# LiHaoxu/SpMV-Research

Measured on AMD Instinct MI355X. Metric: GFLOP/s (2*nnz/t, fp64 SpMV y=A*x); achieved HBM GB/s and % of peak in 'roofline', higher is better.
Workload: dtype f64; 1 GPU; nlpkkt240 (synthetic twin); format=MI355X_SELLD_64_16384_d_v7, rows=27993600, cols=27993600, nnz=765374392, parallelism=single GPU

## Files before the change

### spmv-research_amd/csrc/build_sell.hip

```cpp
#include "handle.hpp"

namespace spmv {

static std::vector<int>
sigma_sort(const int * rp, long m, long sigma)
{
	std::vector<int> row_of_sorted(std::max<long>(m, 1));
	const long num_windows = (m + sigma - 1) / sigma;
	#pragma omp parallel for num_threads(spmv::host_threads()) schedule(dynamic, 4)
	for (long w = 0; w < num_windows; w++)
	{
		long s = w * sigma, e = std::min(m, s + sigma);
		int maxlen = 0;
		for (long i = s; i < e; i++)
			maxlen = std::max(maxlen, rp[i + 1] - rp[i]);
		std::vector<long> cnt((size_t) maxlen + 2, 0);
		for (long i = s; i < e; i++)
			cnt[maxlen - (rp[i + 1] - rp[i]) + 1]++;
		for (int b = 0; b <= maxlen; b++)
			cnt[b + 1] += cnt[b];
		for (long i = s; i < e; i++)
			row_of_sorted[s + cnt[maxlen - (rp[i + 1] - rp[i])]++] = (int) i;
	}
	return row_of_sorted;
// ... 517 lines not shown
			long js = 0, len = 0;
			if (i < m)
			{
				const int o = row_of_sorted[i];
				js = rp[o];
				len = rp[o + 1] - rp[o];
			}
			const unsigned short pad = (len > 0 && !sym) ? (unsigned short) (ci[js + len - 1] - lo) : (unsigned short) gw;
			for (long k = 0; k < width; k++)
			{
				val[(size_t) (vb + sellw_val_pos(k, r, A->f32))] = k < len ? va[js + k] : 0.0;
				idx[(size_t) (ib + (k / 4) * 4 * C + r * 4 + k % 4)] = k < len ? (unsigned short) (ci[js + k] - lo) : pad;
			}
		}
	}
	A->sell_slices = num_slices;
	A->sell_nnz_ext = nnz_ext;
	A->sell_idx_bytes = idx_count * 2;
	A->sellw_groups = (int) num_groups;
	A->sellw_ns = NS;
	A->sell_split = S;
	A->sellw_lds = (int) (((long) (max_w + 1) * A->vbytes + 15) / 16 * 16);
	A->sellw_wmax = max_w;
	{
		std::vector<int64_t> gp((size_t) num_groups + 1, 0);
		for (long g = 0; g < num_groups; g++)
			gp[(size_t) g + 1] = sdesc[2 * std::min<long>(num_slices, (g + 1) * NS)];
		A->cfg.map = xcd_map_balanced(gp.data(), num_groups, 1, resolve_remap(A->remap, num_groups));
	}
	if (upload_ints(grp.data(), grp.size(), &A->d_sellw_grp) || dev_alloc(&A->d_sell_desc, sdesc.size()))
		return 1;
	HIP_TRY(hipMemcpy(A->d_sell_desc, sdesc.data(), sdesc.size() * sizeof(int64_t), hipMemcpyHostToDevice));
	if (upload_bytes(idx.data(), (size_t) idx_count * 2, 1024, (void **) &A->d_sell_idx) || upload_values(A, val.data(), (size_t) nnz_ext, &A->d_val) ||
	    upload_ints(row_of_sorted.data(), (size_t) m, &A->d_row_of_sorted))
		return 1;
	A->mem_footprint = (double) (num_slices + 1) * 16 + (double) num_groups * 16 + (double) nnz_ext * A->vbytes + (double) idx_count * 2 + (double) m * 4;
	return 0;
}

int
build_sell_symmetric(spmv_mi355x_matrix * A, const spmv_mi355x_opts & o, const int * rp, const int * ci, const double * va)
{
	const long lm = A->m;
	const long slices = (lm + 63) / 64;
	const char * pf = A->f32 ? "f" : "d";
	int S = o.sell_split ? o.sell_split : (slices >= 8192 ? 1 : slices >= 2048 ? 2 : 4);
	int NS = o.sell_group ? o.sell_group : 16 / S;
	if ((S != 1 && S != 2 && S != 4) || NS < 1 || NS * S > 16 || (NS & (NS - 1)))
		return 2;
	A->sell_c = 64;
	A->sell_delta = false;
	A->convert_on_device = o.convert_on != 2 && !getenv("SPMV_MI355X_HOST_CONVERT");
	const int took = build_sell_window(A, rp, ci, va, NS, S, 152 * 1024, true);
	if (took)
		return took;
	A->sell_window = true;
	A->sell_sym = true;
	A->sell_sigma = 64L * NS;
	if (o.nontemporal == 0)
		A->cfg.nt = (double) A->sell_nnz_ext * (A->vbytes + 2) > 32.0 * 1024 * 1024 ? 1 : 0;
	if (S > 1)
		snprintf(A->format_name, sizeof(A->format_name), "MI355X_SELLWS_64_%d_w%d_%s", 64 * NS, S, pf);
	else
		snprintf(A->format_name, sizeof(A->format_name), "MI355X_SELLWS_64_%d_%s", 64 * NS, pf);
	snprintf(A->kernel_name, sizeof(A->kernel_name), "sell_window_sym_kernel");
	A->kernel_block = 64 * NS * S;
	return 0;
}

int
build_sell_family(spmv_mi355x_matrix * A, const spmv_mi355x_opts & o, const int * rp, const int * ci, const double * va)
{
	const long lm = A->m;
	const char * pf = A->f32 ? "f" : "d";
	int rc = 0;
	int C = o.sell_c ? o.sell_c : 64;
	if (C != 16 && C != 32 && C != 64 && C != 256)
	{
		set_error("sell_c must be 16, 32, 64 or 256 (got %d)", C);
		return 1;
	}
	long sigma = o.sell_sigma ? o.sell_sigma : 16384;
	if (sigma < C || sigma % C)
	{
		set_error("sell_sigma (%ld) must be a positive multiple of sell_c (%d)", sigma, C);
		return 1;
	}
	A->sell_c = C;
	A->sell_sigma = sigma;
	A->sell_delta = (C == 64) && (o.sell_delta != 2);
	A->convert_on_device = o.convert_on != 2 && !getenv("SPMV_MI355X_HOST_CONVERT");
	{
		const long slices = (lm + 63) / 64;
		int S = o.sell_split ? o.sell_split : (slices >= 16384 ? 1 : slices >= 8192 ? 2 : 4);
		if (S != 1 && S != 2 && S != 4 && !(S == 8 && o.sell_window == 1))
		{
			set_error("sell_split must be 1, 2 or 4 (8 with sell_window = 1) (got %d)", S);
			return 1;
		}
		A->sell_split = A->sell_delta ? S : 1;
	}
	if (o.sell_delta == 1 && C != 64)
	{
		set_error("sell_delta needs sell_c = 64 (one lane per row)");
		return 1;
	}
	if (C == 64 && !A->mixed() && o.sell_window != 2 && (o.sell_window == 1 || (o.sell_delta == 0 && o.convert_on == 0 && o.sell_sigma == 0)))
	{
		const long slices = (lm + 63) / 64;
		const double mean = lm > 0 ? (double) A->nnz / lm : 0;
		int NS = o.sell_group ? o.sell_group : o.sell_sigma ? (int) std::min<long>(16, std::max<long>(1, sigma / 64)) : 0;
		int S = o.sell_split ? o.sell_split : (slices >= 8192 ? 1 : slices >= 2048 ? 2 : 4);
		if (NS == 0)
			NS = 16 / S;
		if (NS < 1 || NS * S > 16 || (NS & (NS - 1)))
		{
			if (o.sell_window == 1)
			{
				set_error("sell_window: %d slices x %d waves per workgroup (a power of two, at most 16 waves)", NS, S);
				return 1;
			}
		}
		else if (o.sell_window == 1 || (mean >= 8 && A->nnz >= (1L << 20) && A->nnz < (1L << 28)))
		{
			const int took = build_sell_window(A, rp, ci, va, NS, S, sell_window_lds_budget());
			if (took == 1)
				return 1;
			if (took == 0)
			{
				A->sell_window = true;
				A->sell_delta = false;
				if (o.nontemporal == 0)
					A->cfg.nt = (double) A->sell_nnz_ext * (A->vbytes + 2) > 32.0 * 1024 * 1024 ? 1 : 0;
				A->sell_sigma = 64L * NS;
				if (S > 1)
					snprintf(A->format_name, sizeof(A->format_name), "MI355X_SELLW_64_%d_w%d_%s", 64 * NS, S, pf);
				else
					snprintf(A->format_name, sizeof(A->format_name), "MI355X_SELLW_64_%d_%s", 64 * NS, pf);
				snprintf(A->kernel_name, sizeof(A->kernel_name), "sell_window_kernel");
				A->kernel_block = 64 * NS * S;
				return 0;
			}
			if (o.sell_window == 1)
			{
				set_error("sell_window: a slice group's column window exceeds 65 536 columns or the LDS budget");
				return 1;
			}
		}
	}
	if (A->sell_delta)
	{
		rc = build_sell_delta(A, sell_values_env(o.sell_values), rp, ci, va);
		A->sell_v7_active = !rc && sell_v7_wanted(A->val_f32, sell_values_env(o.sell_values), A->sell_nnz_ext);
		sell_delta_names(A);
		return rc;
	}
	snprintf(A->format_name, sizeof(A->format_name), "MI355X_SELL_%d_%ld_%s", C, sigma, pf);
	snprintf(A->kernel_name, sizeof(A->kernel_name), "sell_kernel");
	return build_sell(A, rp, ci, va);
}


int
build_sell_delta_resident(spmv_mi355x_matrix * A, const spmv_mi355x_opts & o, const int * d_rp, const int * d_ci, const double * d_va)
{
	constexpr int C = SELL_DELTA_C;
	const long m = A->m;
	if ((o.sell_c && o.sell_c != C) || o.sell_delta == 2 || o.convert_on == 2 || o.sell_window == 1)
	{
		set_error("create_from_stream: only the SELL-64 delta layout converted on the device is built from a device-resident CSR");
		return 1;
	}
	const long sigma = o.sell_sigma ? o.sell_sigma : 16384;
	if (sigma < C || sigma % C)
	{
		set_error("sell_sigma (%ld) must be a positive multiple of sell_c (%d)", sigma, C);
		return 1;
	}
	const long num_slices = (m + C - 1) / C;
	int S = o.sell_split ? o.sell_split : (num_slices >= 16384 ? 1 : num_slices >= 8192 ? 2 : 4);
	if (S != 1 && S != 2 && S != 4)
	{
		set_error("sell_split must be 1, 2 or 4 (got %d)", S);
		return 1;
	}
	A->sell_c = C;
	A->sell_sigma = sigma;
	A->sell_delta = true;
	A->convert_on_device = true;
	A->sell_split = S;
	SellDeltaArrays r;
	if (sell_delta_convert_resident(A->val_f32, m, A->n, A->nnz, sigma, sell_values_env(o.sell_values), d_rp, d_ci, d_va, r))
		return 1;
	sell_delta_install(A, r);
	A->sell_v7_active = sell_v7_wanted(A->val_f32, sell_values_env(o.sell_values), A->sell_nnz_ext);
	sell_delta_names(A);
	return 0;
}

}
```

### spmv-research_amd/csrc/kernels_sell.hip

```cpp

#include <type_traits>

#include "sell_delta_read.hpp"

namespace spmv {

constexpr int SELL_BLOCK = 256;
constexpr int SELL_WAVES = SELL_BLOCK / WAVE;

template <typename T, int C, bool NT>
__global__ __launch_bounds__(SELL_BLOCK) void
sell_kernel(const int64_t * __restrict__ slice_ptr, const int * __restrict__ col, const T * __restrict__ val,
		const int * __restrict__ row_of_sorted, const T * __restrict__ x, T * __restrict__ y,
		int m, int num_slices, int beta, XcdMap map)
{
	unsigned tile = xcd_tile(blockIdx.x, map);
	if (tile == NO_TILE)
		return;
	const int lane = threadIdx.x % WAVE;
	const int slice = tile * SELL_WAVES + threadIdx.x / WAVE;
	if (slice >= num_slices)
		return;
	const int64_t p_s = slice_ptr[slice];
	const int64_t p_e = slice_ptr[slice + 1];
// ... 140 lines not shown
		sell_tail_values<T, NT, NSTEPS>(vals.tail(g), lane, v);
		const T x0 = x[c0];
		const T x1 = NSTEPS > 1 ? x[c1] : T(0);
		const T x2 = NSTEPS > 2 ? x[c2] : T(0);
		s = fma_t<T>(v[0], x0, s);
		if (NSTEPS > 1) s = fma_t<T>(v[1], x1, s);
		if (NSTEPS > 2) s = fma_t<T>(v[2], x2, s);
	}
}

__device__ __forceinline__ void
sell_pin(unsigned & v)
{
	asm volatile("" : "+v"(v));
}
__device__ __forceinline__ void
sell_pin(sell_uint2 & v, bool both)
{
	unsigned a = v.x, b = both ? v.y : 0u;
	asm volatile("" : "+v"(a), "+v"(b));
	v.x = a;
	if (both)
		v.y = b;
}


template <typename T, int MODE, bool NT, bool V7, int NG, typename S = T>
__device__ __forceinline__ void
sell_delta_consume(const SellDeltaIdx<MODE> * q, const SellVals<T, NT, V7, S> & vals, const int * g, const T * __restrict__ x, T & s)
{
	T v[NG][4];
	int c[NG][4];
	T xv[NG][4];
	#pragma unroll
	for (int u = 0; u < NG; u++)
		vals.group(g[u], v[u]);
	#pragma unroll
	for (int u = 0; u < NG; u++)
		sell_delta_cols<MODE>(q[u], c[u]);
	#pragma unroll
	for (int u = 0; u < NG; u++)
		#pragma unroll
		for (int t = 0; t < 4; t++)
			xv[u][t] = x[c[u][t]];
	#pragma unroll
	for (int u = 0; u < NG; u++)
		#pragma unroll
		for (int t = 0; t < 4; t++)
			s = fma_t<T>(v[u][t], xv[u][t], s);
}

template <typename T, int MODE, bool NT, bool V7, typename S = T>
__device__ __forceinline__ void
sell_delta_piped(const unsigned char * __restrict__ ip, const SellVals<T, NT, V7, S> & vals, int lane, const T * __restrict__ x, T & s, int g0, int gs, int n)
{
	constexpr long GB = sell_group_bytes(MODE);
	if (n <= 0)
		return;
	auto gidx = [&](int k) { return g0 + (k < n ? k : n - 1) * gs; };
	SellDeltaIdx<MODE> q[4], nq[4];
	#pragma unroll
	for (int u = 0; u < 4; u++)
		sell_delta_load_idx<MODE, NT>(q[u], ip + (size_t) gidx(u) * GB, lane);
	int k = 0;
	for (; k + 4 <= n; k += 4)
	{
		#pragma unroll
		for (int u = 0; u < 4; u++)
			sell_delta_load_idx<MODE, NT>(nq[u], ip + (size_t) gidx(k + 4 + u) * GB, lane);
		const int g[4] = {gidx(k), gidx(k + 1), gidx(k + 2), gidx(k + 3)};
		sell_delta_consume<T, MODE, NT, V7, 4>(q, vals, g, x, s);
		#pragma unroll
		for (int u = 0; u < 4; u++)
		{
			sell_pin(nq[u].d, MODE == 2);
			q[u] = nq[u];
		}
	}
	const int r = n - k;
	if (r >= 2)
	{
		const int g[2] = {gidx(k), gidx(k + 1)};
		sell_delta_consume<T, MODE, NT, V7, 2>(q, vals, g, x, s);
	}
	if (r == 1)
	{
		const int g[1] = {gidx(k)};
		sell_delta_consume<T, MODE, NT, V7, 1>(q, vals, g, x, s);
	}
	if (r == 3)
	{
		const int g[1] = {gidx(k + 2)};
		sell_delta_consume<T, MODE, NT, V7, 1>(q + 2, vals, g, x, s);
	}
}

template <typename T, int MODE, bool NT, bool V7, typename S = T>
__device__ __forceinline__ T
sell_delta_slice(const unsigned char * __restrict__ ip, const SellVals<T, NT, V7, S> & vals, int width, int lane, const T * __restrict__ x,
		int g0 = 0, int gs = 1)
{
	constexpr long GB = sell_group_bytes(MODE);
	const int groups = (width + 3) / 4;
	const int rem = width - 4 * (groups - 1);
	int off = lane;
	if constexpr (MODE == 3)
	{
		off = ld_stream<NT>(reinterpret_cast<const int *>(ip) + lane);
		ip += sell_header_bytes(3);
	}
	T s = 0;
	int g = g0;
	const int last = groups - 1;
	if constexpr (MODE == 1 || MODE == 2)
	{
		const int full = rem == 4 ? groups : last;
		const int n = full > g0 ? (full - g0 + gs - 1) / gs : 0;
		sell_delta_piped<T, MODE, NT, V7>(ip, vals, lane, x, s, g0, gs, n);
		g = g0 + n * gs;
	}
	const int full_end = rem == 4 ? groups : last;
	for (; g + 3 * gs < full_end; g += 4 * gs)
	{
		sell_delta_group<T, MODE, NT, V7>(ip + (size_t) g * GB, vals, g, lane, x, s, off);
		sell_delta_group<T, MODE, NT, V7>(ip + (size_t) (g + gs) * GB, vals, g + gs, lane, x, s, off);
		sell_delta_group<T, MODE, NT, V7>(ip + (size_t) (g + 2 * gs) * GB, vals, g + 2 * gs, lane, x, s, off);
		sell_delta_group<T, MODE, NT, V7>(ip + (size_t) (g + 3 * gs) * GB, vals, g + 3 * gs, lane, x, s, off);
	}
	for (; g + 2 * gs < full_end; g += 3 * gs)
	{
		sell_delta_group<T, MODE, NT, V7>(ip + (size_t) g * GB, vals, g, lane, x, s, off);
		sell_delta_group<T, MODE, NT, V7>(ip + (size_t) (g + gs) * GB, vals, g + gs, lane, x, s, off);
		sell_delta_group<T, MODE, NT, V7>(ip + (size_t) (g + 2 * gs) * GB, vals, g + 2 * gs, lane, x, s, off);
	}
	for (; g + gs < (rem == 4 ? groups : last); g += 2 * gs)
	{
		sell_delta_group<T, MODE, NT, V7>(ip + (size_t) g * GB, vals, g, lane, x, s, off);
		sell_delta_group<T, MODE, NT, V7>(ip + (size_t) (g + gs) * GB, vals, g + gs, lane, x, s, off);
	}
	for (; g < (rem == 4 ? groups : last); g += gs)
		sell_delta_group<T, MODE, NT, V7>(ip + (size_t) g * GB, vals, g, lane, x, s, off);
	if (rem != 4 && g == last)
	{
		if (rem == 1)
			sell_delta_group<T, MODE, NT, V7, 1>(ip + (size_t) g * GB, vals, g, lane, x, s, off);
		else if (rem == 2)
			sell_delta_group<T, MODE, NT, V7, 2>(ip + (size_t) g * GB, vals, g, lane, x, s, off);
		else
			sell_delta_group<T, MODE, NT, V7, 3>(ip + (size_t) g * GB, vals, g, lane, x, s, off);
	}
	return s;
}


template <bool SCALAR>
__device__ __forceinline__ void
sell_pin5(SellDeltaIdx5 & q)
{
	if constexpr (SCALAR)
	{
		int a = q.corr.x, b = q.corr.y, c = q.corr.z, d = q.corr.w;
		asm volatile("" : "+s"(a), "+s"(b), "+s"(c), "+s"(d));
		q.corr.x = a;
		q.corr.y = b;
		q.corr.z = c;
		q.corr.w = d;
	}
	else
		sell_pin(q.d);
}

template <typename T, bool NT, bool V7, bool SCALAR, typename S = T>
__device__ __forceinline__ T
sell_delta_slice5_body(const unsigned char * __restrict__ ip, const SellVals<T, NT, V7, S> & vals, int width, int lane, const T * __restrict__ x,
		int g0, int gs, unsigned long long mask, int off)
{
	const int E = __popcll(mask);
	const bool ex = (mask >> lane) & 1ull;
	const int rank = ex ? __popcll(mask & ((1ull << lane) - 1ull)) : 0;
	int xl[4] = {0, 0, 0, 0};
	if constexpr (SCALAR)
	{
		unsigned long long mm = mask;
		const int spare = __builtin_ctzll(~mask);
		#pragma unroll
		for (int j = 0; j < 4; j++)
		{
			xl[j] = mm ? __builtin_ctzll(mm) : spare;
			mm &= mm - 1ull;
		}
	}
	const size_t GB = sell_group_bytes(5, E);
	const int groups = (width + 3) / 4;
	const int rem = width - 4 * (groups - 1);
	const int last = groups - 1;
	const int full = rem == 4 ? groups : last;
	const int n = full > g0 ? (full - g0 + gs - 1) / gs : 0;
	T s = 0;
	if (n > 0)
	{
		auto gidx = [&](int k) { return g0 + (k < n ? k : n - 1) * gs; };
		auto consume = [&](const SellDeltaIdx5 * q, const int * g, auto ng) {
			constexpr int NG = decltype(ng)::value;
			T v[NG][4];
			int c[NG][4];
			T xv[NG][4];
			#pragma unroll
			for (int u = 0; u < NG; u++)
				vals.group(g[u], v[u]);
			#pragma unroll
			for (int u = 0; u < NG; u++)
				sell_delta_cols5<SCALAR>(q[u], ex, lane, off, xl, c[u]);
			#pragma unroll
			for (int u = 0; u < NG; u++)
				#pragma unroll
				for (int t = 0; t < 4; t++)
					xv[u][t] = x[c[u][t]];
			#pragma unroll
			for (int u = 0; u < NG; u++)
				#pragma unroll
				for (int t = 0; t < 4; t++)
					s = fma_t<T>(v[u][t], xv[u][t], s);
		};
		SellDeltaIdx5 q[4], nq[4];
		#pragma unroll
		for (int u = 0; u < 4; u++)
			sell_delta_load_idx5<NT, SCALAR>(q[u], ip + (size_t) gidx(u) * GB, rank);
		int k = 0;
		for (; k + 4 <= n; k += 4)
		{
			#pragma unroll
			for (int u = 0; u < 4; u++)
				sell_delta_load_idx5<NT, SCALAR>(nq[u], ip + (size_t) gidx(k + 4 + u) * GB, rank);
			const int g[4] = {gidx(k), gidx(k + 1), gidx(k + 2), gidx(k + 3)};
			consume(q, g, std::integral_constant<int, 4>());
			#pragma unroll
			for (int u = 0; u < 4; u++)
			{
				sell_pin5<SCALAR>(nq[u]);
				q[u] = nq[u];
			}
		}
		const int r = n - k;
		if (r >= 2)
		{
			const int g[2] = {gidx(k), gidx(k + 1)};
			consume(q, g, std::integral_constant<int, 2>());
		}
		if (r == 1)
		{
			const int g[1] = {gidx(k)};
			consume(q, g, std::integral_constant<int, 1>());
		}
		if (r == 3)
		{
			const int g[1] = {gidx(k + 2)};
			consume(q + 2, g, std::integral_constant<int, 1>());
		}
	}
	if (rem != 4 && last >= g0 && (last - g0) % gs == 0)
	{
		SellDeltaIdx5 q;
		sell_delta_load_idx5<NT, SCALAR>(q, ip + (size_t) last * GB, rank);
		int c[4];
		sell_delta_cols5<SCALAR>(q, ex, lane, off, xl, c);
		const S * vl = vals.tail(last);
		T tv[3];
		if (rem == 1)
			sell_tail_values<T, NT, 1>(vl, lane, tv);
		else if (rem == 2)
			sell_tail_values<T, NT, 2>(vl, lane, tv);
		else
			sell_tail_values<T, NT, 3>(vl, lane, tv);
		const T v0 = tv[0], v1 = tv[1], v2 = tv[2];
		const T x0 = x[c[0]];
		const T x1 = rem > 1 ? x[c[1]] : T(0);
		const T x2 = rem > 2 ? x[c[2]] : T(0);
		s = fma_t<T>(v0, x0, s);
		if (rem > 1) s = fma_t<T>(v1, x1, s);
		if (rem > 2) s = fma_t<T>(v2, x2, s);
	}
	return s;
}

template <typename T, bool NT, bool V7, typename S = T>
__device__ __forceinline__ T
sell_delta_slice5(const unsigned char * __restrict__ ip, const SellVals<T, NT, V7, S> & vals, int width, int lane, const T * __restrict__ x,
		int g0 = 0, int gs = 1)
{
	const int off = ld_stream<NT>(reinterpret_cast<const int *>(ip) + lane);
	const unsigned long long mask = *reinterpret_cast<const unsigned long long *>(ip + 4 * WAVE);
	ip += sell_header_bytes(5);
	if (__popcll(mask) <= 4)
		return sell_delta_slice5_body<T, NT, V7, true>(ip, vals, width, lane, x, g0, gs, mask, off);
	return sell_delta_slice5_body<T, NT, V7, false>(ip, vals, width, lane, x, g0, gs, mask, off);
}

template <typename T, bool NT, bool V7, typename S = T>
__device__ __forceinline__ T
sell_delta_modes(int mode, const unsigned char * __restrict__ ip, const SellVals<T, NT, V7, S> & vals, int width, int lane, const T * __restrict__ x,
		int g0, int gs)
{
	if (mode == 0)
		return sell_delta_slice<T, 0, NT>(ip, vals, width, lane, x, g0, gs);
	if (mode == 1)
		return sell_delta_slice<T, 1, NT>(ip, vals, width, lane, x, g0, gs);
	if (mode == 2)
		return sell_delta_slice<T, 2, NT>(ip, vals, width, lane, x, g0, gs);
	if (mode == 3)
		return sell_delta_slice<T, 3, NT>(ip, vals, width, lane, x, g0, gs);
	if (mode == 5)
		return sell_delta_slice5<T, NT>(ip, vals, width, lane, x, g0, gs);
	return sell_delta_slice<T, 4, NT>(ip, vals, width, lane, x, g0, gs);
}

template <typename T, bool NT, bool V7, typename S = T>
__device__ __forceinline__ T
sell_delta_one(const int64_t * __restrict__ desc, int slice, const unsigned char * __restrict__ idx, const S * __restrict__ val, int lane,
		const T * __restrict__ x, int g0, int gs)
{
	const int64_t v_off = desc[2 * slice];
	const int64_t i_word = desc[2 * slice + 1];
	const int64_t v_next = desc[2 * slice + 2];
	const int mode = sell_desc_mode(i_word);
	const unsigned char * ip = idx + sell_desc_idx(i_word);
	const S * vp = val + v_off + 2 * lane;
	if (V7 && sell_desc_v7(i_word))
		return sell_delta_modes<T, NT, V7>(mode, ip, SellVals<T, NT, V7, S>{vp, lane, (unsigned) (sell_v7_e0(i_word) - 1) << 20},
				(int) sell_slice_width(v_next - v_off, true), lane, x, g0, gs);
	return sell_delta_modes<T, NT, false>(mode, ip, SellVals<T, NT, false, S>{vp, lane, 0u}, (int) sell_slice_width(v_next - v_off, false), lane, x,
			g0, gs);
}

static_assert(SELL_WAVES % SELL_DELTA_WAVES == 0, "the handle's tiles are whole numbers of sell_delta_kernel's");
template <typename T> constexpr int sell_delta_waves() { return sizeof(T) == 8 ? SELL_DELTA_WAVES : SELL_WAVES; }

template <int W>
static XcdMap
sell_delta_tile_map(const XcdMap & mp, int num_slices)
{
	constexpr unsigned F = SELL_WAVES / W;
	XcdMap o = mp;
	o.ntiles = ((unsigned) num_slices + W - 1) / W;
	o.chunk = mp.chunk * F;
	for (int k = 0; k < NUM_XCD; k++)
		o.start[k] = mp.start[k] * F < o.ntiles ? mp.start[k] * F : o.ntiles;
	o.start[NUM_XCD] = o.ntiles;
	return o;
}

template <typename T, bool NT, bool V7, int W = sell_delta_waves<T>()>
__global__ __launch_bounds__(W * WAVE) void
sell_delta_kernel(const int64_t * __restrict__ desc, const unsigned char * __restrict__ idx, const T * __restrict__ val,
		const int * __restrict__ row_of_sorted, const T * __restrict__ x, T * __restrict__ y,
		int m, int num_slices, int beta, XcdMap map)
{
	unsigned tile = xcd_tile(blockIdx.x, map);
	if (tile == NO_TILE)
		return;
	const int lane = threadIdx.x % WAVE;
	const int slice = __builtin_amdgcn_readfirstlane((int) (tile * W + threadIdx.x / WAVE));
	if (slice >= num_slices)
		return;
	const T s = sell_delta_one<T, NT, V7>(desc, slice, idx, val, lane, x, 0, 1);
	const long sorted_row = (long) slice * WAVE + lane;
	if (sorted_row < m)
	{
		T * yp = y + row_of_sorted[sorted_row];
		*yp = beta ? *yp + s : s;
	}
}

template <typename T, int S, bool NT, bool V7>
__global__ __launch_bounds__(SELL_BLOCK) void
sell_delta_split_kernel(const int64_t * __restrict__ desc, const unsigned char * __restrict__ idx, const T * __restrict__ val,
		const int * __restrict__ row_of_sorted, const T * __restrict__ x, T * __restrict__ y,
		int m, int num_slices, int beta, XcdMap map)
{
	constexpr int SPB = SELL_WAVES / S;
	__shared__ T s_part[SELL_WAVES][WAVE];
	unsigned tile = xcd_tile(blockIdx.x, map);
	if (tile == NO_TILE)
		return;
	const int lane = threadIdx.x % WAVE;
	const int wave = threadIdx.x / WAVE;
	const int w = __builtin_amdgcn_readfirstlane(wave % S);
	const int slice = __builtin_amdgcn_readfirstlane((int) (tile * SPB + wave / S));
	T s = 0;
	if (slice < num_slices)
		s = sell_delta_one<T, NT, V7>(desc, slice, idx, val, lane, x, w, S);
	s_part[wave][lane] = s;
	__syncthreads();
	if (w == 0 && slice < num_slices)
	{
		T t = s_part[wave][lane];
		#pragma unroll
		for (int u = 1; u < S; u++)
			t += s_part[wave + u][lane];
		const long sorted_row = (long) slice * WAVE + lane;
		if (sorted_row < m)
		{
			T * yp = y + row_of_sorted[sorted_row];
			*yp = beta ? *yp + t : t;
		}
	}
}

template <bool NT>
__global__ __launch_bounds__(SELL_BLOCK) void
sell_delta_mixed_kernel(const int64_t * __restrict__ desc, const unsigned char * __restrict__ idx, const float * __restrict__ val,
		const int * __restrict__ row_of_sorted, const double * __restrict__ x, double * __restrict__ y,
		int m, int num_slices, int beta, XcdMap map)
{
	unsigned tile = xcd_tile(blockIdx.x, map);
	if (tile == NO_TILE)
		return;
	const int lane = threadIdx.x % WAVE;
	const int slice = __builtin_amdgcn_readfirstlane((int) (tile * SELL_WAVES + threadIdx.x / WAVE));
	if (slice >= num_slices)
		return;
	const double s = sell_delta_one<double, NT, false>(desc, slice, idx, val, lane, x, 0, 1);
	const long sorted_row = (long) slice * WAVE + lane;
	if (sorted_row < m)
	{
		double * yp = y + row_of_sorted[sorted_row];
		*yp = beta ? *yp + s : s;
	}
}

template <int S, bool NT>
__global__ __launch_bounds__(SELL_BLOCK) void
sell_delta_mixed_split_kernel(const int64_t * __restrict__ desc, const unsigned char * __restrict__ idx, const float * __restrict__ val,
		const int * __restrict__ row_of_sorted, const double * __restrict__ x, double * __restrict__ y,
		int m, int num_slices, int beta, XcdMap map)
{
	constexpr int SPB = SELL_WAVES / S;
	__shared__ double s_part[SELL_WAVES][WAVE];
	unsigned tile = xcd_tile(blockIdx.x, map);
	if (tile == NO_TILE)
		return;
	const int lane = threadIdx.x % WAVE;
	const int wave = threadIdx.x / WAVE;
	const int w = __builtin_amdgcn_readfirstlane(wave % S);
	const int slice = __builtin_amdgcn_readfirstlane((int) (tile * SPB + wave / S));
	double s = 0;
	if (slice < num_slices)
		s = sell_delta_one<double, NT, false>(desc, slice, idx, val, lane, x, w, S);
	s_part[wave][lane] = s;
	__syncthreads();
	if (w == 0 && slice < num_slices)
	{
		double t = s_part[wave][lane];
		#pragma unroll
		for (int u = 1; u < S; u++)
			t += s_part[wave + u][lane];
		const long sorted_row = (long) slice * WAVE + lane;
		if (sorted_row < m)
		{
			double * yp = y + row_of_sorted[sorted_row];
			*yp = beta ? *yp + t : t;
		}
	}
}

template <typename T, bool V7, bool MIXED = false>
static int
sell_delta_launch(int S, const int64_t * desc, const unsigned char * idx, const void * val, const int * row_of_sorted, const void * x, void * y,
		int m, int num_slices, const LaunchCfg & cfg, hipStream_t stream, long * grid_out)
{
	unsigned grid = xcd_grid(cfg.map);
	if (grid_out)
		*grid_out = grid;
	if (grid == 0)
		return 0;
	typedef std::conditional_t<MIXED, float, T> SV;
	#define SELLD_LAUNCH(K) hipLaunchKernelGGL(K, dim3(grid), dim3(SELL_BLOCK), 0, stream, desc, idx, (const SV *) val, \
			row_of_sorted, (const T *) x, (T *) y, m, num_slices, cfg.beta, cfg.map)
	if (S != 1 && S != 2 && S != 4)
	{
		set_error("sell_delta: waves per slice must be 1, 2 or 4 (got %d)", S);
		return 1;
	}
	if constexpr (MIXED)
	{
		static_assert(std::is_same<T, double>::value && !V7, "fp32 values under fp64 vectors, plain pairs");
		if (S == 1)
		{
			if (cfg.nt) SELLD_LAUNCH((sell_delta_mixed_kernel<true>));
			else        SELLD_LAUNCH((sell_delta_mixed_kernel<false>));
		}
		else if (S == 2)
		{
			if (cfg.nt) SELLD_LAUNCH((sell_delta_mixed_split_kernel<2, true>));
			else        SELLD_LAUNCH((sell_delta_mixed_split_kernel<2, false>));
		}
		else
		{
			if (cfg.nt) SELLD_LAUNCH((sell_delta_mixed_split_kernel<4, true>));
			else        SELLD_LAUNCH((sell_delta_mixed_split_kernel<4, false>));
		}
	}
	else if (S == 1)
	{
		constexpr int W = sell_delta_waves<T>();
		const XcdMap map1 = sell_delta_tile_map<W>(cfg.map, num_slices);
		grid = xcd_grid(map1);
		if (grid_out)
			*grid_out = grid;
		#define SELLD_LAUNCH1(K) hipLaunchKernelGGL(K, dim3(grid), dim3(W * WAVE), 0, stream, desc, idx, (const T *) val, \
				row_of_sorted, (const T *) x, (T *) y, m, num_slices, cfg.beta, map1)
		if (cfg.nt) SELLD_LAUNCH1((sell_delta_kernel<T, true, V7>));
		else        SELLD_LAUNCH1((sell_delta_kernel<T, false, V7>));
		#undef SELLD_LAUNCH1
	}
	else if (S == 2)
	{
		if (cfg.nt) SELLD_LAUNCH((sell_delta_split_kernel<T, 2, true, V7>));
		else        SELLD_LAUNCH((sell_delta_split_kernel<T, 2, false, V7>));
	}
	else
	{
		if (cfg.nt) SELLD_LAUNCH((sell_delta_split_kernel<T, 4, true, V7>));
		else        SELLD_LAUNCH((sell_delta_split_kernel<T, 4, false, V7>));
	}
	#undef SELLD_LAUNCH
	HIP_TRY(hipGetLastError());
	return 0;
}

int
launch_sell_delta(bool f32, bool val_f32, int waves_per_slice, bool v7, const int64_t * desc, const unsigned char * idx, const void * val, const int * row_of_sorted,
		const void * x, void * y, int m, int num_slices, const LaunchCfg & cfg, hipStream_t stream, long * grid_out)
{
	if (val_f32 && v7)
	{
		set_error("sell_delta: 7-byte values are fp64 only");
		return 1;
	}
	if (f32 && !val_f32)
	{
		set_error("sell_delta: fp32 vectors over fp64 values are not served");
		return 1;
	}
	if (val_f32 && !f32)
		return sell_delta_launch<double, false, true>(waves_per_slice, desc, idx, val, row_of_sorted, x, y, m, num_slices, cfg, stream, grid_out);
	return f32 ? sell_delta_launch<float, false>(waves_per_slice, desc, idx, val, row_of_sorted, x, y, m, num_slices, cfg, stream, grid_out)
	     : v7  ? sell_delta_launch<double, true>(waves_per_slice, desc, idx, val, row_of_sorted, x, y, m, num_slices, cfg, stream, grid_out)
	           : sell_delta_launch<double, false>(waves_per_slice, desc, idx, val, row_of_sorted, x, y, m, num_slices, cfg, stream, grid_out);
}

template <typename T, int C>
static int
sell_launch_c(const int64_t * slice_ptr, const int * col, const void * val, const int * row_of_sorted, const void * x, void * y,
		int m, int num_slices, const LaunchCfg & cfg, hipStream_t stream, long * grid_out)
{
	unsigned grid = xcd_grid(cfg.map);
	if (grid_out)
		*grid_out = grid;
	if (grid == 0)
		return 0;
	if (cfg.nt)
		hipLaunchKernelGGL((sell_kernel<T, C, true>), dim3(grid), dim3(SELL_BLOCK), 0, stream, slice_ptr, col, (const T *) val,
				row_of_sorted, (const T *) x, (T *) y, m, num_slices, cfg.beta, cfg.map);
	else
		hipLaunchKernelGGL((sell_kernel<T, C, false>), dim3(grid), dim3(SELL_BLOCK), 0, stream, slice_ptr, col, (const T *) val,
				row_of_sorted, (const T *) x, (T *) y, m, num_slices, cfg.beta, cfg.map);
	HIP_TRY(hipGetLastError());
	return 0;
}

template <typename T>
static int
sell_dispatch(int C, const int64_t * slice_ptr, const int * col, const void * val, const int * row_of_sorted, const void * x, void * y,
		int m, int num_slices, const LaunchCfg & cfg, hipStream_t stream, long * grid_out)
{
	if (C == SELL_WIDE_C)
	{
		const unsigned grid = xcd_grid(cfg.map);
		if (grid_out)
			*grid_out = grid;
		if (grid == 0)
			return 0;
		if (cfg.nt)
			hipLaunchKernelGGL((sell_wide_kernel<T, true>), dim3(grid), dim3(SELL_WIDE_C), 0, stream, slice_ptr, col, (const T *) val, row_of_sorted,
					(const T *) x, (T *) y, m, num_slices, cfg.beta, cfg.map);
		else
			hipLaunchKernelGGL((sell_wide_kernel<T, false>), dim3(grid), dim3(SELL_WIDE_C), 0, stream, slice_ptr, col, (const T *) val, row_of_sorted,
					(const T *) x, (T *) y, m, num_slices, cfg.beta, cfg.map);
		HIP_TRY(hipGetLastError());
		return 0;
	}
	switch (C)
	{
		case 16: return sell_launch_c<T, 16>(slice_ptr, col, val, row_of_sorted, x, y, m, num_slices, cfg, stream, grid_out);
		case 32: return sell_launch_c<T, 32>(slice_ptr, col, val, row_of_sorted, x, y, m, num_slices, cfg, stream, grid_out);
		case 64: return sell_launch_c<T, 64>(slice_ptr, col, val, row_of_sorted, x, y, m, num_slices, cfg, stream, grid_out);
	}
	set_error("sell: C must be 16, 32, 64 or 256 (got %d)", C);
	return 1;
}

int
launch_sell(bool f32, int C, const int64_t * slice_ptr, const int * col, const void * val, const int * row_of_sorted,
		const void * x, void * y, int m, int num_slices, const LaunchCfg & cfg, hipStream_t stream, long * grid_out)
{
	return f32 ? sell_dispatch<float>(C, slice_ptr, col, val, row_of_sorted, x, y, m, num_slices, cfg, stream, grid_out)
	           : sell_dispatch<double>(C, slice_ptr, col, val, row_of_sorted, x, y, m, num_slices, cfg, stream, grid_out);
}

}
```

### spmv-research_amd/csrc/launch.hpp

```cpp
#pragma once

#include <vector>

#include "common.hpp"
#include "sell_delta_layout.hpp"

namespace spmv {

struct LaunchCfg {
	XcdMap map;
	int nt;
	int beta;
	int unit;
	double unit_value;
	int kahan;
};

inline long csr_scalar_rows_per_tile() { return 256; }
inline long csr_vector_rows_per_tile(int lanes_per_row, int rows_per_group = 1) { return 256L / lanes_per_row * rows_per_group; }
inline long csr_stream_rows_per_tile(int rows_per_wave) { return 4L * rows_per_wave; }
inline long sell_slices_per_tile() { return 4; }
constexpr int SELL_DELTA_WAVES = 1;
inline long coo_waves_per_tile() { return 4; }

int launch_csr_scalar(bool f32, const int * row_ptr, const int * col, const void * val, const void * x, void * y,
		int m, const LaunchCfg & cfg, hipStream_t stream, long * grid_out);
int launch_csr_vector(bool f32, int lanes_per_row, int rows_per_group, const int * row_ptr, const int * col, const void * val,
		const void * x, void * y, int m, const LaunchCfg & cfg, hipStream_t stream, long * grid_out);

int csr_stream_cap();
int launch_csr_stream(bool f32, int rows_per_wave, const int * row_ptr, const int * col, const void * val, const void * x, void * y,
		int m, const LaunchCfg & cfg, hipStream_t stream, long * grid_out);

int csr_stream_t_cap(int rows_per_wave);
int launch_csr_stream_t(bool f32, int rows_per_wave, const int * row_ptr, const int * col, const void * val, const void * x, void * y,
		int m, const LaunchCfg & cfg, hipStream_t stream, long * grid_out);

int csr_stream_d_cap(int rows_per_wave);
long csr_stream_d_rows_per_tile(int rows_per_wave);
int launch_csr_stream_d(bool f32, int rows_per_wave, const int * row_ptr, const int * col, const void * val, const void * x, void * y,
		int m, const LaunchCfg & cfg, hipStream_t stream, long * grid_out);
constexpr int STREAM_SLACK = 512;

int csr_window_lds_budget();
int launch_csr_window(bool f32, int lanes_per_row, const int * row_ptr, const void * col, int col16, const void * val, const void * x, void * y,
		const int * blk_row, const int * blk_lo, const int * blk_w, int lds_bytes, const LaunchCfg & cfg, hipStream_t stream,
		long * grid_out);

int merge_tile_items(bool f32, int items_per_thread);
int launch_merge_search(const int * row_ptr, int m, int nnz, int tile_items, int num_tiles, int * coords ,
		hipStream_t stream);
int launch_merge(bool f32, int items_per_thread, const int * row_ptr, const int * col, const void * val, const void * x, void * y,
		int m, int nnz, int num_tiles, const int * coords, int * carry_row, void * carry_val,
		const LaunchCfg & cfg, hipStream_t stream, long * grid_out);

int launch_sell(bool f32, int C, const int64_t * slice_ptr, const int * col, const void * val, const int * row_of_sorted,
		const void * x, void * y, int m, int num_slices, const LaunchCfg & cfg, hipStream_t stream, long * grid_out);

int launch_sell_delta(bool f32, bool val_f32, int waves_per_slice, bool v7, const int64_t * desc, const unsigned char * idx, const void * val, const int * row_of_sorted,
		const void * x, void * y, int m, int num_slices, const LaunchCfg & cfg, hipStream_t stream, long * grid_out);

int launch_sell_delta_spmm(bool f32, bool val_f32, int waves_per_slice, bool v7, const int64_t * desc, const unsigned char * idx, const void * val,
		const int * row_of_sorted, int k, const void * X, long ldx, void * Y, long ldy, int m, int num_slices, const LaunchCfg & cfg,
		hipStream_t stream, long * grid_out);
inline int
spmm_pass_cols(int cap, int remaining)
{
	int K = 1;
	while (2 * K <= cap && 2 * K <= remaining)
		K *= 2;
	return K;
}
constexpr int SELL_DELTA_SPMM_COLS = 8;
int launch_spmm_column_gather(bool f32, const void * X, long ldx, void * x, long n, hipStream_t stream);
int launch_spmm_column_scatter(bool f32, const void * y, void * Y, long ldy, long m, int beta, hipStream_t stream);

int sell_window_lds_budget();
int launch_sell_window(bool f32, int waves_per_slice, int slices_per_group, const int * grp, const int64_t * sdesc, const unsigned short * idx,
		const void * val, const int * row_of_sorted, const void * x, void * y, int m, int lds_window_bytes, const LaunchCfg & cfg,
		hipStream_t stream, long * grid_out);

int sell_window_spmm_max_cols(bool f32, int waves_per_slice, int slices_per_group, int wmax);
int launch_sell_window_spmm(bool f32, int waves_per_slice, int slices_per_group, const int * grp, const int64_t * sdesc, const unsigned short * idx,
		const void * val, const int * row_of_sorted, int k, const void * X, long ldx, void * Y, long ldy, int m, int wmax, const LaunchCfg & cfg,
		hipStream_t stream, long * grid_out);

int launch_sell_window_sym(bool f32, int waves_per_slice, int slices_per_group, const int * grp, const int64_t * sdesc, const unsigned short * idx,
		const void * val, const int * row_of_sorted, const void * x, void * y, int m, int lds_window_bytes, const LaunchCfg & cfg,
		hipStream_t stream, long * grid_out);

inline int
sell_modes_off()
{
	const char * e = getenv("SPMV_MI355X_SELL_MODES_OFF");
	return e ? atoi(e) & 7 : 0;
}

inline int
sell_values_env(int opt)
{
	const char * e = getenv("SPMV_MI355X_SELL_VALUES");
	return e ? atoi(e) : opt;
}

__host__ __device__ inline long
sellw_val_pos(long k, long r, bool f32)
{
	return f32 ? (k / 4) * 256 + r * 4 + (k & 3) : (k / 2) * 128 + r * 2 + (k & 1);
}

struct SellDeltaArrays {
	int * row_of_sorted = nullptr;
	int64_t * desc = nullptr;
	unsigned char * idx = nullptr;
	void * val = nullptr;
	std::vector<int64_t> val_ptr;
	long mode_counts[4] = {0, 0, 0, 0};
	int64_t nnz_ext = 0;
	int64_t idx_bytes = 0;
	int64_t val_words = 0;
	long v7_slices = 0;
};

int sell_delta_convert_device(bool f32, long m, long n_cols, long nnz, long sigma, int sell_values, const int * rp_host, const int * ci_host,
		const double * va_host, SellDeltaArrays & out);

int sell_delta_convert_resident(bool f32, long m, long n_cols, long nnz, long sigma, int sell_values, const int * rp, const int * ci,
		const double * va, SellDeltaArrays & out);
int blocked_entries_convert_device(bool f32, bool uniform, long m, long nnz, const int * rp_host, const int * ci_host, const double * va_host, long NR, int WGS, long CH,
		const std::vector<int> & range_row, const std::vector<int> & range_long, const std::vector<int> & long_row, const std::vector<int> & chunk_ptr,
		const std::vector<int> & chunk_row, const std::vector<int> & wg_rows, long SPAN, long BATCH, int slot_bits, int SPARE, long ghost_batches,
		std::vector<int> & batch_ptr, unsigned ** d_ent_out, void ** d_val_out, int ** d_batch_base_out);
int sell_plain_convert_device(bool f32, long m, long nnz, int C, int TPR, long sigma, const int * rp_host, const int * ci_host, const double * va_host,
		int64_t ** d_slice_ptr_out, int ** d_col_out, void ** d_val_out, int ** d_row_of_sorted_out, std::vector<int64_t> & slice_ptr_host);
int sell_window_convert_device(bool f32, long m, long nnz, int NS, bool sym, long lds_budget_bytes, const int * rp_host, const int * ci_host,
		const double * va_host, int ** d_grp_out, int ** d_row_of_sorted_out, int64_t ** d_desc_out, unsigned short ** d_idx_out, void ** d_val_out,
		std::vector<int64_t> & desc_host, int * max_w_out);

int coo_wave_items(int items_per_lane);
int launch_coo(bool f32, int items_per_lane, const int * rowind, const int * col, const void * val, const void * x, void * y,
		int m, long nnz, int num_waves, int * carry_row, void * carry_val,
		const LaunchCfg & cfg, hipStream_t stream, long * grid_out);

int coo_blocked_rows_cap(bool f32);
int coo_blocked_wgs_per_range();
int coo_blocked_chunk_rows();
int coo_blocked_batch_entries(bool unit);
int coo_blocked_spare_slots();
int coo_blocked_slot_bits();
int coo_blocked_max_long_rows();
int launch_coo_blocked(bool f32, const int * wg_rows, const int * range_row, const int * chunk_ptr, const int * chunk_row, const int * batch_ptr, const int * batch_base,
		const int * range_long,
		const int * long_row, int num_long, const unsigned * ent, const void * val, const void * x, void * y, void * carry, int num_ranges,
		int chunk_rows, int lds_bytes, const LaunchCfg & cfg, hipStream_t stream, long * grid_out);

int launch_expand_rows(const int * row_ptr, int m, int * rowind, hipStream_t stream);

}
```

### spmv-research_amd/csrc/sell_delta_read.hpp

```cpp
#pragma once

#include "launch.hpp"

namespace spmv {

typedef int sell_int4 __attribute__((ext_vector_type(4)));
typedef unsigned sell_uint2 __attribute__((ext_vector_type(2)));

template <typename T, bool NT, typename S = T>
__device__ __forceinline__ void
sell_group_values(const S * __restrict__ vp, T (&v)[4])
{
	typedef S S2 __attribute__((ext_vector_type(2)));
	const S2 w0 = ld_stream<NT>(reinterpret_cast<const S2 *>(vp));
	const S2 w1 = ld_stream<NT>(reinterpret_cast<const S2 *>(vp + 2 * WAVE));
	v[0] = w0.x;
	v[1] = w0.y;
	v[2] = w1.x;
	v[3] = w1.y;
}

template <typename T, bool NT, int NSTEPS, typename S = T>
__device__ __forceinline__ void
sell_tail_values(const S * __restrict__ vp, int lane, T (&v)[3])
// ... 27 lines not shown
	int lane;
	unsigned k;
	__device__ __forceinline__ void group(int g, T (&v)[4]) const
	{
		if constexpr (!V7)
			sell_group_values<T, NT, S>(vp + (size_t) g * 4 * WAVE, v);
		else
		{
			static_assert(sizeof(T) == 8 && sizeof(S) == 8, "7-byte values are fp64 only");
			const unsigned char * b = reinterpret_cast<const unsigned char *>(vp) + (size_t) g * (8 * SELL_V7_GROUP_WORDS);
			const sell_uint4 lo = ld_stream<NT>(reinterpret_cast<const sell_uint4 *>(b));
			const sell_uint3 * hp = reinterpret_cast<const sell_uint3 *>(b + 1024 - 4 * lane);
			sell_uint3 hi;
			if constexpr (NT)
				hi = __builtin_nontemporal_load(hp);
			else
				hi = *hp;
			v[0] = sell_v7_value(hi.x, k, lo.x);
			v[1] = sell_v7_value(__builtin_amdgcn_alignbit(hi.y, hi.x, 24), k, lo.y);
			v[2] = sell_v7_value(__builtin_amdgcn_alignbit(hi.z, hi.y, 16), k, lo.z);
			v[3] = sell_v7_value(hi.z >> 8, k, lo.w);
		}
	}
	__device__ __forceinline__ const S * tail(int g) const { return vp + (size_t) g * (V7 ? SELL_V7_GROUP_WORDS : 4 * WAVE); }
};

template <int MODE>
struct SellDeltaIdx {
	sell_int4 base;
	sell_uint2 d;
};

template <int MODE, bool NT>
__device__ __forceinline__ void
sell_delta_load_idx(SellDeltaIdx<MODE> & q, const unsigned char * __restrict__ gp , int lane)
{
	q.base = *reinterpret_cast<const sell_int4 *>(gp);
	if constexpr (MODE == 1)
		q.d.x = ld_stream<NT>(reinterpret_cast<const unsigned *>(gp + 16) + lane);
	else
		q.d = ld_stream<NT>(reinterpret_cast<const sell_uint2 *>(gp + 16) + lane);
}

template <int MODE>
__device__ __forceinline__ void
sell_delta_cols(const SellDeltaIdx<MODE> & q, int (&c)[4])
{
	if constexpr (MODE == 1)
	{
		c[0] = q.base.x + (int) (q.d.x & 255u);
		c[1] = q.base.y + (int) ((q.d.x >> 8) & 255u);
		c[2] = q.base.z + (int) ((q.d.x >> 16) & 255u);
		c[3] = q.base.w + (int) (q.d.x >> 24);
	}
	else
	{
		c[0] = q.base.x + (int) (q.d.x & 0xffffu);
		c[1] = q.base.y + (int) (q.d.x >> 16);
		c[2] = q.base.z + (int) (q.d.y & 0xffffu);
		c[3] = q.base.w + (int) (q.d.y >> 16);
	}
}

struct SellDeltaIdx5 {
	sell_int4 base;
	unsigned d;
	sell_int4 corr;
};

template <bool NT, bool SCALAR>
__device__ __forceinline__ void
sell_delta_load_idx5(SellDeltaIdx5 & q, const unsigned char * __restrict__ gp , int rank)
{
	q.base = *reinterpret_cast<const sell_int4 *>(gp);
	if constexpr (SCALAR)
		q.corr = *reinterpret_cast<const sell_int4 *>(gp + 16);
	else
		q.d = ld_stream<NT>(reinterpret_cast<const unsigned *>(gp + 16) + rank);
}

template <bool SCALAR>
__device__ __forceinline__ void
sell_delta_cols5(const SellDeltaIdx5 & q, bool ex, int lane, int off, const int (&xl)[4], int (&c)[4])
{
	int d;
	if constexpr (SCALAR)
	{
		d = lane == xl[0] ? q.corr.x : 0;
		d = lane == xl[1] ? q.corr.y : d;
		d = lane == xl[2] ? q.corr.z : d;
		d = lane == xl[3] ? q.corr.w : d;
	}
	else
		d = ex ? (int) q.d : 0;
	c[0] = q.base.x + off + ((d << 24) >> 24);
	c[1] = q.base.y + off + ((d << 16) >> 24);
	c[2] = q.base.z + off + ((d << 8) >> 24);
	c[3] = q.base.w + off + (d >> 24);
}

template <int MODE, bool NT>
__device__ __forceinline__ void
sell_group_cols(const unsigned char * __restrict__ gp , int lane, int off, int (&c)[4])
{
	static_assert(MODE >= 0 && MODE <= 4, "mode 5 has its own reader (sell_delta_load_idx5, sell_delta_cols5)");
	if constexpr (MODE == 0 || MODE == 3)
	{
		const sell_int4 base = *reinterpret_cast<const sell_int4 *>(gp);
		c[0] = base.x + off;
		c[1] = base.y + off;
		c[2] = base.z + off;
		c[3] = base.w + off;
	}
	else if constexpr (MODE == 1 || MODE == 2)
	{
		SellDeltaIdx<MODE> q;
		sell_delta_load_idx<MODE, NT>(q, gp, lane);
		sell_delta_cols<MODE>(q, c);
	}
	else
	{
		const int * cp = reinterpret_cast<const int *>(gp) + lane;
		c[0] = ld_stream<NT>(cp);
		c[1] = ld_stream<NT>(cp + WAVE);
		c[2] = ld_stream<NT>(cp + 2 * WAVE);
		c[3] = ld_stream<NT>(cp + 3 * WAVE);
	}
}

template <bool SCALAR>
struct Sell5Lane {
	bool ex;
	int rank;
	int xl[4];
	__device__ __forceinline__ Sell5Lane(unsigned long long mask, int lane)
	{
		ex = (mask >> lane) & 1ull;
		rank = ex ? __popcll(mask & ((1ull << lane) - 1ull)) : 0;
		xl[0] = xl[1] = xl[2] = xl[3] = 0;
		if constexpr (SCALAR)
		{
			unsigned long long mm = mask;
			const int spare = __builtin_ctzll(~mask);
			#pragma unroll
			for (int j = 0; j < 4; j++)
			{
				xl[j] = mm ? __builtin_ctzll(mm) : spare;
				mm &= mm - 1ull;
			}
		}
	}
};

}
```

Baseline: 1435 GFLOP/s.

## Reuse x values across consecutive-column groups via DPP lane shift in SELL delta kernel

Adds a 'runs' path for SELL delta slices in modes 0 and 3, where column = base_k + lane offset. When a group's base is the previous base plus one, each lane's x value equals the neighbour lane's previous x value. That value is obtained with a DPP wave rotate instead of a fresh gather, and only lane 63 loads a new element. The aim is to cut x gather traffic and load instructions on banded matrices such as nlpkkt240. In exchange it adds cross-lane dependencies, extra registers for the batched unrolled loads, and a pre-check ballot for mode 3. It is enabled by default for fp64 through an environment variable.

```diff
diff --git a/spmv-research_amd/csrc/build_sell.hip b/spmv-research_amd/csrc/build_sell.hip
--- a/spmv-research_amd/csrc/build_sell.hip
+++ b/spmv-research_amd/csrc/build_sell.hip
@@ -693,6 +693,7 @@
 	{
 		rc = build_sell_delta(A, sell_values_env(o.sell_values), rp, ci, va);
 		A->sell_v7_active = !rc && sell_v7_wanted(A->val_f32, sell_values_env(o.sell_values), A->sell_nnz_ext);
+		A->cfg.sell_runs = sell_runs_env();
 		sell_delta_names(A);
 		return rc;
 	}
@@ -735,6 +736,7 @@
 		return 1;
 	sell_delta_install(A, r);
 	A->sell_v7_active = sell_v7_wanted(A->val_f32, sell_values_env(o.sell_values), A->sell_nnz_ext);
+	A->cfg.sell_runs = sell_runs_env();
 	sell_delta_names(A);
 	return 0;
 }
diff --git a/spmv-research_amd/csrc/kernels_sell.hip b/spmv-research_amd/csrc/kernels_sell.hip
--- a/spmv-research_amd/csrc/kernels_sell.hip
+++ b/spmv-research_amd/csrc/kernels_sell.hip
@@ -316,6 +316,83 @@
 	return s;
 }
 
+
+template <typename T, bool NT, bool V7, int NG>
+__device__ __forceinline__ void
+sell_runs_trip(const unsigned char * __restrict__ gp , const SellVals<T, NT, V7> & vals, int g, const T * __restrict__ x, T & s, int off,
+		int off63, unsigned & pb, T & px)
+{
+	T v[NG][4], xl[NG][4], xs[NG][4];
+	bool run[NG][4];
+	#pragma unroll
+	for (int u = 0; u < NG; u++)
+	{
+		const sell_int4 base = *reinterpret_cast<const sell_int4 *>(gp + u * 16);
+		const int b[4] = {base.x, base.y, base.z, base.w};
+		vals.group(g + u, v[u]);
+		#pragma unroll
+		for (int t = 0; t < 4; t++)
+		{
+			run[u][t] = (unsigned) b[t] - pb == 1u;
+			pb = (unsigned) b[t];
+			xs[u][t] = x[b[t] + off63];
+			xl[u][t] = sell_unset();
+			if (!run[u][t])
+				xl[u][t] = x[b[t] + off];
+		}
+	}
+	#pragma unroll
+	for (int u = 0; u < NG; u++)
+		#pragma unroll
+		for (int t = 0; t < 4; t++)
+		{
+			const T moved = sell_lane_up(xs[u][t], px);
+			px = run[u][t] ? moved : xl[u][t];
+			s = fma_t<T>(v[u][t], px, s);
+		}
+}
+
+template <typename T, int MODE, bool NT, bool V7>
+__device__ __forceinline__ T
+sell_runs_slice(const unsigned char * __restrict__ ip, const SellVals<T, NT, V7> & vals, int width, int lane, const T * __restrict__ x)
+{
+	static_assert(MODE == 0 || MODE == 3, "the modes whose columns are base_k + off_l");
+	constexpr long GB = sell_group_bytes(MODE);
+	int off = lane, off63 = WAVE - 1;
+	if constexpr (MODE == 3)
+	{
+		off = ld_stream<NT>(reinterpret_cast<const int *>(ip) + lane);
+		if (__ballot(sell_lane_broken(off, lane)) != 1ull << (WAVE - 1))
+			return sell_delta_slice<T, 3, NT>(ip, vals, width, lane, x);
+		ip += sell_header_bytes(3);
+		off63 = __builtin_amdgcn_readlane(off, WAVE - 1);
+	}
+	const int groups = (width + 3) / 4;
+	const int rem = width - 4 * (groups - 1);
+	const int last = groups - 1;
+	const int full_end = rem == 4 ? groups : last;
+	T s = 0, px = 0;
+	unsigned pb = full_end > 0 ? *reinterpret_cast<const unsigned *>(ip) : 0u;
+	int g = 0;
+	for (; g + 3 < full_end; g += 4)
+		sell_runs_trip<T, NT, V7, 4>(ip + (size_t) g * GB, vals, g, x, s, off, off63, pb, px);
+	for (; g + 2 < full_end; g += 3)
+		sell_runs_trip<T, NT, V7, 3>(ip + (size_t) g * GB, vals, g, x, s, off, off63, pb, px);
+	for (; g + 1 < full_end; g += 2)
+		sell_runs_trip<T, NT, V7, 2>(ip + (size_t) g * GB, vals, g, x, s, off, off63, pb, px);
+	for (; g < full_end; g++)
+		sell_runs_trip<T, NT, V7, 1>(ip + (size_t) g * GB, vals, g, x, s, off, off63, pb, px);
+	if (rem != 4)
+	{
+		if (rem == 1)
+			sell_delta_group<T, MODE, NT, V7, 1>(ip + (size_t) last * GB, vals, last, lane, x, s, off);
+		else if (rem == 2)
+			sell_delta_group<T, MODE, NT, V7, 2>(ip + (size_t) last * GB, vals, last, lane, x, s, off);
+		else
+			sell_delta_group<T, MODE, NT, V7, 3>(ip + (size_t) last * GB, vals, last, lane, x, s, off);
+	}
+	return s;
+}
 
 template <bool SCALAR>
 __device__ __forceinline__ void
@@ -460,11 +537,18 @@
 	return sell_delta_slice5_body<T, NT, V7, false>(ip, vals, width, lane, x, g0, gs, mask, off);
 }
 
-template <typename T, bool NT, bool V7, typename S = T>
+template <typename T, bool NT, bool V7, typename S = T, bool RUNS = false>
 __device__ __forceinline__ T
 sell_delta_modes(int mode, const unsigned char * __restrict__ ip, const SellVals<T, NT, V7, S> & vals, int width, int lane, const T * __restrict__ x,
 		int g0, int gs)
 {
+	if constexpr (RUNS)
+	{
+		if (mode == 0)
+			return sell_runs_slice<T, 0, NT>(ip, vals, width, lane, x);
+		if (mode == 3)
+			return sell_runs_slice<T, 3, NT>(ip, vals, width, lane, x);
+	}
 	if (mode == 0)
 		return sell_delta_slice<T, 0, NT>(ip, vals, width, lane, x, g0, gs);
 	if (mode == 1)
@@ -478,7 +562,7 @@
 	return sell_delta_slice<T, 4, NT>(ip, vals, width, lane, x, g0, gs);
 }
 
-template <typename T, bool NT, bool V7, typename S = T>
+template <typename T, bool NT, bool V7, typename S = T, bool RUNS = false>
 __device__ __forceinline__ T
 sell_delta_one(const int64_t * __restrict__ desc, int slice, const unsigned char * __restrict__ idx, const S * __restrict__ val, int lane,
 		const T * __restrict__ x, int g0, int gs)
@@ -490,9 +574,9 @@
 	const unsigned char * ip = idx + sell_desc_idx(i_word);
 	const S * vp = val + v_off + 2 * lane;
 	if (V7 && sell_desc_v7(i_word))
-		return sell_delta_modes<T, NT, V7>(mode, ip, SellVals<T, NT, V7, S>{vp, lane, (unsigned) (sell_v7_e0(i_word) - 1) << 20},
+		return sell_delta_modes<T, NT, V7, S, RUNS>(mode, ip, SellVals<T, NT, V7, S>{vp, lane, (unsigned) (sell_v7_e0(i_word) - 1) << 20},
 				(int) sell_slice_width(v_next - v_off, true), lane, x, g0, gs);
-	return sell_delta_modes<T, NT, false>(mode, ip, SellVals<T, NT, false, S>{vp, lane, 0u}, (int) sell_slice_width(v_next - v_off, false), lane, x,
+	return sell_delta_modes<T, NT, false, S, RUNS>(mode, ip, SellVals<T, NT, false, S>{vp, lane, 0u}, (int) sell_slice_width(v_next - v_off, false), lane, x,
 			g0, gs);
 }
 
@@ -513,7 +597,7 @@
 	return o;
 }
 
-template <typename T, bool NT, bool V7, int W = sell_delta_waves<T>()>
+template <typename T, bool NT, bool V7, int W = sell_delta_waves<T>(), bool RUNS = false>
 __global__ __launch_bounds__(W * WAVE) void
 sell_delta_kernel(const int64_t * __restrict__ desc, const unsigned char * __restrict__ idx, const T * __restrict__ val,
 		const int * __restrict__ row_of_sorted, const T * __restrict__ x, T * __restrict__ y,
@@ -526,7 +610,7 @@
 	const int slice = __builtin_amdgcn_readfirstlane((int) (tile * W + threadIdx.x / WAVE));
 	if (slice >= num_slices)
 		return;
-	const T s = sell_delta_one<T, NT, V7>(desc, slice, idx, val, lane, x, 0, 1);
+	const T s = sell_delta_one<T, NT, V7, T, RUNS>(desc, slice, idx, val, lane, x, 0, 1);
 	const long sorted_row = (long) slice * WAVE + lane;
 	if (sorted_row < m)
 	{
@@ -673,8 +757,18 @@
 			*grid_out = grid;
 		#define SELLD_LAUNCH1(K) hipLaunchKernelGGL(K, dim3(grid), dim3(W * WAVE), 0, stream, desc, idx, (const T *) val, \
 				row_of_sorted, (const T *) x, (T *) y, m, num_slices, cfg.beta, map1)
-		if (cfg.nt) SELLD_LAUNCH1((sell_delta_kernel<T, true, V7>));
-		else        SELLD_LAUNCH1((sell_delta_kernel<T, false, V7>));
+		if constexpr (sizeof(T) == 8)
+		{
+			if (cfg.sell_runs)
+			{
+				if (cfg.nt) SELLD_LAUNCH1((sell_delta_kernel<T, true, V7, W, true>));
+				else        SELLD_LAUNCH1((sell_delta_kernel<T, false, V7, W, true>));
+			}
+			else if (cfg.nt) SELLD_LAUNCH1((sell_delta_kernel<T, true, V7>));
+			else             SELLD_LAUNCH1((sell_delta_kernel<T, false, V7>));
+		}
+		else if (cfg.nt) SELLD_LAUNCH1((sell_delta_kernel<T, true, V7>));
+		else             SELLD_LAUNCH1((sell_delta_kernel<T, false, V7>));
 		#undef SELLD_LAUNCH1
 	}
 	else if (S == 2)
diff --git a/spmv-research_amd/csrc/launch.hpp b/spmv-research_amd/csrc/launch.hpp
--- a/spmv-research_amd/csrc/launch.hpp
+++ b/spmv-research_amd/csrc/launch.hpp
@@ -14,6 +14,7 @@
 	int unit;
 	double unit_value;
 	int kahan;
+	int sell_runs;
 };
 
 inline long csr_scalar_rows_per_tile() { return 256; }
@@ -97,6 +98,13 @@
 }
 
 inline int
+sell_runs_env()
+{
+	const char * e = getenv("SPMV_MI355X_SELL_RUNS");
+	return e ? atoi(e) != 0 : 1;
+}
+
+inline int
 sell_values_env(int opt)
 {
 	const char * e = getenv("SPMV_MI355X_SELL_VALUES");
diff --git a/spmv-research_amd/csrc/sell_delta_read.hpp b/spmv-research_amd/csrc/sell_delta_read.hpp
--- a/spmv-research_amd/csrc/sell_delta_read.hpp
+++ b/spmv-research_amd/csrc/sell_delta_read.hpp
@@ -203,4 +203,27 @@
 	}
 };
 
-}
+__device__ __forceinline__ double
+sell_lane_up(double keep, double v)
+{
+	const unsigned long long k = __builtin_bit_cast(unsigned long long, keep), w = __builtin_bit_cast(unsigned long long, v);
+	const unsigned lo = (unsigned) __builtin_amdgcn_update_dpp((int) (unsigned) k, (int) (unsigned) w, 0x130, 0xf, 0xf, false);
+	const unsigned hi = (unsigned) __builtin_amdgcn_update_dpp((int) (unsigned) (k >> 32), (int) (unsigned) (w >> 32), 0x130, 0xf, 0xf, false);
+	return __builtin_bit_cast(double, (unsigned long long) hi << 32 | lo);
+}
+
+__device__ __forceinline__ double
+sell_unset()
+{
+	unsigned lo, hi;
+	asm("" : "=v"(lo), "=v"(hi));
+	return __builtin_bit_cast(double, (unsigned long long) hi << 32 | lo);
+}
+
+__device__ __forceinline__ bool
+sell_lane_broken(int off, int lane)
+{
+	return lane == WAVE - 1 || (unsigned) __shfl_down(off, 1) - (unsigned) off != 1u;
+}
+
+}
```

Measured after the change: 1451 GFLOP/s, median of 5. +1.1%, better.
